# nv-dvl/nerfmatch

Hardware: AMD Instinct MI355X
Metric: rays*samples/sec (higher is better)
Workload: dtype fp16x3 (fp16 MFMA on hi/lo-split fp32 operands, three products per fp32 product, fp32 accumulate; fp32 everywhere else)

## Files before the change

### nerfmatch_amd/csrc/nerf_fwd_bf16.hip

```cpp
#include "nerf_split_chain.h"

namespace {
using namespace nmbf;

template <int PART>
__device__ __forceinline__ void tap_prefetch(Ctx& cx) {
  if constexpr (PART == 0) __builtin_amdgcn_s_barrier();
  const char* src = reinterpret_cast<const char*>(cx.tapw);
#pragma unroll
  for (int q = (PART == 0 ? 0 : 4); q < (PART == 0 ? 4 : 7); ++q) {
    const char* sp = src + q * 4096;
    const float* dp = q < 4 ? cx.tap_ring + q * 1024 : cx.tap_ipe + (q - 4) * 1024;
    const unsigned lds = (unsigned)__builtin_amdgcn_readfirstlane((int)(unsigned)(size_t)(const __attribute__((address_space(3))) float*)dp);
    unsigned m0_saved;
    asm volatile("s_mov_b32 %0, m0\n\ts_mov_b32 m0, %1\n\tglobal_load_lds_dwordx4 %2, off\n\tglobal_load_lds_dwordx4 %2, off offset:1024\n\t"
                 "global_load_lds_dwordx4 %2, off offset:2048\n\tglobal_load_lds_dwordx4 %2, off offset:3072\n\ts_mov_b32 m0, %0"
                 : "=&s"(m0_saved) : "s"(lds), "v"(sp) : "memory");
  }
}

__device__ __forceinline__ void dpp_pairs8(float (&o)[8], const float (&x)[8], const float (&y)[8], bool eight) {
  if (eight)
    asm("s_nop 1\n"
        "v_add_f32_dpp %0, %8, %8 row_mirror row_mask:0xf bank_mask:0x3\n\tv_add_f32_dpp %1, %9, %9 row_mirror row_mask:0xf bank_mask:0x3\n\t"
// ... 166 lines not shown
  const float o0 = rp[0], o1 = rp[1], o2 = rp[2], d0 = rp[3], d1 = rp[4], d2 = rp[5], radius = rp[11];
  const float dsq0 = d0 * d0, dsq1 = d1 * d1, dsq2 = d2 * d2;
  const float dmag = fmaxf(1e-10f, (dsq0 + dsq1) + dsq2);
  const float dnorm = sqrtf((dsq0 + dsq1) + dsq2);
  const float nul0 = 1.0f - dsq0 / dmag, nul1 = 1.0f - dsq1 / dmag, nul2 = 1.0f - dsq2 / dmag;

  float red_acc = 0.f;
  float carryT = 1.f;
  float best_w = -1.f;
  float feat_run = 0.f;

  const int nch = lo_pass ? 1 : nchunks;
  for (int chunk = 0; chunk < nch; ++chunk) {
    const int sidx = lo_pass ? Sa : chunk * TILE + (js % SP);
    const float t0 = a.t[(size_t)rc * (S + 1) + sidx];
    const float t1 = a.t[(size_t)rc * (S + 1) + sidx + 1];
    const float mu = (t0 + t1) / 2.0f, hw = (t1 - t0) / 2.0f;
    const float mu2 = mu * mu, hw2 = hw * hw, hw4 = hw2 * hw2;
    const float denom = fmaxf(1.1920928955078125e-07f, 3.0f * mu2 + hw2);
    const float t_mean = mu + (2.0f * mu * hw2) / denom;
    const float t_var = hw2 / 3.0f - (float)(4.0 / 15.0) * ((hw4 * (12.0f * mu2 - hw2)) / (denom * denom));
    const float r_var = (radius * radius) * ((mu2 / 4.0f + (float)(5.0 / 12.0) * hw2) - (float)(4.0 / 15.0) * hw4 / denom);
    float mean[3] = {d0 * t_mean + o0, d1 * t_mean + o1, d2 * t_mean + o2};
    float var[3] = {t_var * dsq0 + r_var * nul0, t_var * dsq1 + r_var * nul1, t_var * dsq2 + r_var * nul2};
    if (a.var_scale > 0.f) {
      var[0] *= a.var_scale; var[1] *= a.var_scale; var[2] *= a.var_scale;
    }
    if (hi == 0) {
      sm_t0[js] = t0; sm_t1[js] = t1;
      sm_mean[js] = mean[0]; sm_mean[TILE + js] = mean[1]; sm_mean[2 * TILE + js] = mean[2];
      sm_dn[js] = dnorm;
    }

#pragma unroll
    for (int g0 = 0; g0 < ring_ahead<P>(); ++g0) dma_slot<P>(blob_slots, g0, ring, wave, lane);

    {
      float* dst = sm_ipe + wave * (XS * 2 * 64 * 4) + lane * 4;
      const float ipe_scale = sm_small[OFF_INSCALE];
      const float phl = hi ? 1.57079637050628662109375f : 0.f;
#pragma unroll
      for (int m = 0; m < XS; ++m) {
        float v8[8];
#pragma unroll
        for (int i = 0; i < 8; ++i) {
          const int idx = 8 * m + i;
          const bool live = idx < 45;
          const int ax = (live ? idx : 0) % 3, sb = (live ? idx : 0) / 3;
          const float mu = mean[ax], vr = var[ax];
          const float sc = (float)(1 << sb);
          const float xe = mu * sc;
          float v = __builtin_amdgcn_exp2f((-0.5f * (vr * (sc * sc))) * 1.44269504088896340736f) * sin32(xe + phl);
          if constexpr (P == 2) v *= ipe_scale;
          v8[i] = live ? v : 0.f;
        }
        if constexpr (is_split<P>()) {
          bf16x8 h8, l8;
          split8_p<P>(v8, h8, l8);
          *reinterpret_cast<u32x4*>(dst + (m * 2 + 0) * 256) = __builtin_bit_cast(u32x4, h8);
          *reinterpret_cast<u32x4*>(dst + (m * 2 + 1) * 256) = __builtin_bit_cast(u32x4, l8);
        } else {
          *reinterpret_cast<u32x4*>(dst + m * 256) = __builtin_bit_cast(u32x4, pack8_f16(v8));
        }
      }
    }

    TRACE(2);
    Ctx cx;
    cx.blob_slots = blob_slots; cx.ring = ring; cx.sm_small = sm_small;
    cx.tapw = reinterpret_cast<f32x4*>(a.ws) + ((size_t)blockIdx.x * 4 + wave) * 32 * 64 + lane;
    cx.nslots = nslots; cx.wave = wave; cx.lane = lane; cx.hi = hi; cx.tap = need_tap ? tap : -1; cx.g = 0; cx.sig_part = 0.f;
    cx.vmax = 0.f; cx.rng = sm_rng + tid; cx.sc = 1.f;
    const bool early = need_rgb && !lo_pass && tap == 7 && a.feat && !a.sfeat;
    cx.tap_pref = need_tap && !lo_pass && !early; cx.rgb = need_rgb;
    cx.tap_ring = ring + wave * SLOT_FLOATS; cx.tap_ipe = sm_ipe + wave * (XS * 2 * 64 * 4);
    if constexpr (is_split<P>()) {
      NM_WAIT_VMCNT(8);
      __builtin_amdgcn_s_barrier();
    } else {
      ring_acquire<P>(blob_slots, 0, nslots, ring, wave, lane);
    }
    load_half<P>(cx.opA, ring, lane, 0);
    if constexpr (P == 1) load_half<1>(cx.opB, ring, lane, 1);
    const float* ipe_src = sm_ipe + wave * (XS * 2 * 64 * 4) + lane * 4;

    auto composite_weights = [&]() __attribute__((always_inline)) {
      const int tid2 = launder(threadIdx.x), lane2 = tid2 & 63, wave2 = tid2 >> 6;
      float alpha = 0.f, incl = 1.f;
      if (tid2 < TILE) {
        const float sg = fmaxf(sm_sigma[tid2], 0.f);
        const float delta = (sm_t1[tid2] - sm_t0[tid2]) * sm_dn[tid2];
        alpha = 1.0f - expf(-sg * delta);
        incl = (1.0f - alpha) + 1e-10f;
        const int seg = SP < 64 ? SP : 64;
#pragma unroll
        for (int dlt = 1; dlt < 64; dlt <<= 1) {
          const float up = __shfl_up(incl, dlt, 64);
          if (dlt < seg && (lane2 & (seg - 1)) >= dlt) incl *= up;
        }
        if (lane2 == 63) sm_misc[wave2] = incl;
      }
      NM_EPI_BARRIER();
      if (tid2 < TILE) {
        const int seg = SP < 64 ? SP : 64;
        float excl = __shfl_up(incl, 1, 64);
        if ((lane2 & (seg - 1)) == 0) excl = 1.f;
        if (SP == TILE && wave2 == 1) excl *= sm_misc[0];
        excl *= carryT;
        sm_w[tid2] = alpha * excl;
        const int r2 = tid2 / SP, ray2 = bid * nr + r2;
        if (left && chunk == nchunks - 1 && ray2 < R && tid2 % SP == SP - 1) {
// ... 102 lines not shown
      views_hidden<P>(av, cx);
      fold_range<P>(cx, 7);
      bf16x8 exh[VS], exl[VS];
#pragma unroll
      for (int e = 0; e < VS; ++e) {
        float v8[8];
        if (!lo_pass) {
          const f32x4 e0 = *reinterpret_cast<const f32x4*>(exr + 16 * e), e1 = *reinterpret_cast<const f32x4*>(exr + 16 * e + 4);
          v8[0] = e0[0]; v8[1] = e0[1]; v8[2] = e0[2]; v8[3] = e0[3]; v8[4] = e1[0]; v8[5] = e1[1]; v8[6] = e1[2]; v8[7] = e1[3];
        } else {
          const float* rq = a.rays + (size_t)launder(rc) * 12 + 8;
          const float vd0 = rq[0], vd1 = rq[1], vd2 = rq[2];
#pragma unroll
          for (int i = 0; i < 8; ++i) {
            const int f = 16 * e + 8 * hh + i;
            const int ax = f % 3;
            const float dax = ax == 0 ? vd0 : ax == 1 ? vd1 : vd2;
            float v = 0.f;
            if (f < 24) {
              const float xe = dax * (float)(1 << ((f % 12) / 3));
              v = nm_sinf(f < 12 ? xe : xe + 1.57079637050628662109375f);
            } else if (f < 27) {
              v = dax;
            } else if (f < 43) {
              v = a.app_row ? a.app_row[f - 27] : 0.f;
            }
            if constexpr (P == 2) v *= sm_small[OFF_INSCALE + (f < 27 ? 1 : 2)];
            v8[i] = v;
          }
        }
        if constexpr (is_split<P>()) split8_p<P>(v8, exh[e], exl[e]);
        else exh[e] = exl[e] = pack8_f16(v8);
      }
      views_extras<P>(av, cx, exh, exl);
      TRACE(11);
      NM_MLP_DONE_WAIT();
      if (cx.tap_pref) tap_prefetch<0>(cx);
      const float* bv = sm_small + OFF_BVIEWS + 4 * hh;
      const float* wr = sm_small + OFF_WRGB + 4 * hh;
      float pr = 0.f, pg = 0.f, pb = 0.f;
#pragma unroll
      for (int ob = 0; ob < 4; ++ob) {
#pragma unroll
        for (int q = 0; q < 4; ++q) {
          const f32x4 b4 = *reinterpret_cast<const f32x4*>(bv + ob * 32 + 8 * q);
          const f32x4 wr4 = *reinterpret_cast<const f32x4*>(wr + ob * 32 + 8 * q);
          const f32x4 wg4 = *reinterpret_cast<const f32x4*>(wr + 128 + ob * 32 + 8 * q);
          const f32x4 wb4 = *reinterpret_cast<const f32x4*>(wr + 256 + ob * 32 + 8 * q);
#pragma unroll
          for (int e = 0; e < 4; ++e) {
            const float hv = __builtin_fmaxf(acc_read(av[ob][4 * q + e]) + b4[e], 0.f);
            pr = NM_FMA(hv, wr4[e], pr);
            pg = NM_FMA(hv, wg4[e], pg);
            pb = NM_FMA(hv, wb4[e], pb);
          }
        }
      }
      pr = (pr + nm_shfl_xor32(pr)) + sm_small[OFF_MISC + 1];
      pg = (pg + nm_shfl_xor32(pg)) + sm_small[OFF_MISC + 2];
      pb = (pb + nm_shfl_xor32(pb)) + sm_small[OFF_MISC + 3];
      c_r = 1.0f / (1.0f + expf(-pr));
      c_g = 1.0f / (1.0f + expf(-pg));
      c_b = 1.0f / (1.0f + expf(-pb));
      if (cx.tap_pref) tap_prefetch<1>(cx);
    }
    const float sigma_raw = (cx.sig_part + nm_shfl_xor32(cx.sig_part)) + sm_small[OFF_MISC];
    TRACE(12);
// ... 240 lines not shown
```

### nerfmatch_amd/csrc/nerf_points_bf16.hip

```cpp
#include "nerf_split_chain.h"

namespace {
using namespace nmbf;

struct PointsArgs {
  const char* blob;
  const float* xi;
  const float* xd;
  const float* g4;
  float* out4;
  float* g_xi0;
  float* g_xi5;
  float* g_xd;
  u32x4* gates;
  int n, ntiles;
  const float* rays;
  const float* z;
  const float* app_row;
  int S, Sa;
  float* feats;
  const float* tap_w;
  const float* tap_g;
  int tap;
};

__device__ __forceinline__ void dump_tap_rows(int lo, const Ctx& cx, float* dst_row, int hh, bool valid) {
  const float* bl = cx.sm_small + OFF_BIAS + lo * 256 + 4 * hh;
  auto* tp = (__attribute__((address_space(1))) f32x4*)(dst_row + 4 * hh);
#pragma unroll
  for (int ob = 0; ob < 8; ++ob)
#pragma unroll
    for (int q = 0; q < 4; ++q) {
      const f32x4 b = *reinterpret_cast<const f32x4*>(bl + ob * 32 + 8 * q);
      f32x4 v;
#pragma unroll
      for (int e = 0; e < 4; ++e) v[e] = __builtin_fmaxf(cx.hv[ob * 16 + 4 * q + e] + b[e], 0.f);
      if (valid) tp[ob * 8 + q * 2] = v;
    }
}

template <int P, bool RAYS>
__device__ __forceinline__ void points_fwd_body(const PointsArgs& a) {
  __shared__ __attribute__((aligned(16))) float sm[LDS_SCR];
  float* const sm_small = sm + LDS_SMALL;
  float* const ring = sm + LDS_RING;
  float* const sm_ipe = sm + LDS_IPE;
  const int tid = threadIdx.x, lane = tid & 63, wave = tid >> 6, s = lane & 31, hi = lane >> 5;
  const char* const blob_slots = a.blob + (size_t)SMALL_PAD * 4;
  for (int i = tid; i < SMALL / 4; i += 256) reinterpret_cast<f32x4*>(sm_small)[i] = reinterpret_cast<const f32x4*>(a.blob)[i];
#pragma unroll 1
  for (int bid = blockIdx.x; bid < a.ntiles; bid += gridDim.x) {
    __syncthreads();
    const int sample = bid * TILE + wave * 32 + s;
    const size_t sc = (size_t)(sample < a.n ? sample : a.n - 1);
#pragma unroll
    for (int g0 = 0; g0 < ring_ahead<P>(); ++g0) dma_slot<P>(blob_slots, g0, ring, wave, lane);
    float vdir[3] = {0.f, 0.f, 0.f};
    {
      float* dst = sm_ipe + wave * (XS * 2 * 64 * 4) + lane * 4;
      if constexpr (RAYS) {
        const int r = (int)(sc / (size_t)a.Sa), si = (int)(sc % (size_t)a.Sa);
        const float* rp = a.rays + (size_t)r * 12;
        const float t0 = a.z[(size_t)r * (a.S + 1) + si], t1 = a.z[(size_t)r * (a.S + 1) + si + 1];
        const float d0 = rp[3], d1 = rp[4], d2 = rp[5], radius = rp[11];
        vdir[0] = rp[8]; vdir[1] = rp[9]; vdir[2] = rp[10];
        const float mu = (t0 + t1) / 2.0f, hw = (t1 - t0) / 2.0f;
        const float mu2 = mu * mu, hw2 = hw * hw, hw4 = hw2 * hw2;
        const float denom = fmaxf(1.1920928955078125e-07f, 3.0f * mu2 + hw2);
        const float t_mean = mu + (2.0f * mu * hw2) / denom;
        const float t_var = hw2 / 3.0f - (float)(4.0 / 15.0) * ((hw4 * (12.0f * mu2 - hw2)) / (denom * denom));
        const float r_var = (radius * radius) * ((mu2 / 4.0f + (float)(5.0 / 12.0) * hw2) - (float)(4.0 / 15.0) * hw4 / denom);
        const float dsq[3] = {d0 * d0, d1 * d1, d2 * d2};
        const float dmag = fmaxf(1e-10f, (dsq[0] + dsq[1]) + dsq[2]);
        float mean[3], var[3];
#pragma unroll
        for (int ax = 0; ax < 3; ++ax) {
          mean[ax] = rp[ax] + t_mean * vdir[ax];
          var[ax] = t_var * dsq[ax] + r_var * (1.0f - dsq[ax] / dmag);
        }
        const float phl = hi ? 1.57079637050628662109375f : 0.f;
#pragma unroll
        for (int m = 0; m < XS; ++m) {
          float v8[8];
#pragma unroll
          for (int i = 0; i < 8; ++i) {
            const int idx = 8 * m + i;
            const bool live = idx < 45;
            const int ax = (live ? idx : 0) % 3, sb = (live ? idx : 0) / 3;
            const float scl = (float)(1 << sb);
            const float xe = mean[ax] * scl;
            const float v = expf(-0.5f * (var[ax] * (scl * scl))) * nm_sinf(xe + phl);
            v8[i] = live ? v : 0.f;
          }
          bf16x8 h8, l8;
          split8_p<P>(v8, h8, l8);
          *reinterpret_cast<u32x4*>(dst + (m * 2 + 0) * 256) = __builtin_bit_cast(u32x4, h8);
          *reinterpret_cast<u32x4*>(dst + (m * 2 + 1) * 256) = __builtin_bit_cast(u32x4, l8);
        }
      } else {
        const float* row = a.xi + sc * 96 + 45 * hi;
#pragma unroll
        for (int m = 0; m < XS; ++m) {
          float v8[8];
#pragma unroll
          for (int i = 0; i < 8; ++i) v8[i] = (8 * m + i) < 45 ? row[8 * m + i] : 0.f;
          bf16x8 h8, l8;
          split8_p<P>(v8, h8, l8);
          *reinterpret_cast<u32x4*>(dst + (m * 2 + 0) * 256) = __builtin_bit_cast(u32x4, h8);
          *reinterpret_cast<u32x4*>(dst + (m * 2 + 1) * 256) = __builtin_bit_cast(u32x4, l8);
        }
      }
    }
    Ctx cx;
    cx.blob_slots = blob_slots; cx.ring = ring; cx.sm_small = sm_small; cx.tapw = nullptr;
    cx.nslots = NSLOT_FULL; cx.wave = wave; cx.lane = lane; cx.hi = hi; cx.tap = -1; cx.g = 0; cx.sig_part = 0.f;
    cx.vmax = 0.f; cx.rng = nullptr; cx.sc = 1.f; cx.tap_pref = false; cx.rgb = true; cx.tap_ring = nullptr; cx.tap_ipe = nullptr;
    cx.gptr = a.gates + (size_t)bid * 9 * 256 + tid;
    cx.gbits[0] = cx.gbits[1] = cx.gbits[2] = cx.gbits[3] = 0u;
    NM_WAIT_VMCNT(8);
    __builtin_amdgcn_s_barrier();
    load_half<P>(cx.opA, ring, lane, 0);
    const float* ipe_src = sm_ipe + wave * (XS * 2 * 64 * 4) + lane * 4;
    f32x16 acc[8];
    ipe_steps<P, true>(acc, cx, ipe_src);
    finish_layer<P>(acc, 0, cx);
    const bool tapped = a.feats != nullptr;
#pragma unroll 1
    for (int l = 1; l < 8; ++l) {
      if (tapped && l - 1 == a.tap) dump_tap_rows(l - 1, cx, a.feats + sc * 256, launder(lane) >> 5, sample < a.n);
      layer_pass<P>(acc, l, cx, ipe_src);
    }
    if (tapped && a.tap == 7) dump_tap_rows(7, cx, a.feats + sc * 256, launder(lane) >> 5, sample < a.n);
    f32x16 av[4];
    views_hidden<P>(av, cx);
    cx.gptr[7 * 256] = u32x4{cx.gbits[0], cx.gbits[1], cx.gbits[2], cx.gbits[3]};
    const int hh = launder(lane) >> 5;
    {
      const float* row = a.xd + sc * 48 + 8 * hh;
      bf16x8 exh[VS], exl[VS];
#pragma unroll
      for (int e = 0; e < VS; ++e) {
        float v8[8];
        if constexpr (RAYS) {
#pragma unroll
          for (int i = 0; i < 8; ++i) {
            const int f = 16 * e + 8 * hh + i;
            const int ax = f % 3;
            const float dax = ax == 0 ? vdir[0] : ax == 1 ? vdir[1] : vdir[2];
            float v = 0.f;
            if (f < 24) {
              const float xe = dax * (float)(1 << ((f % 12) / 3));
              v = nm_sinf(f < 12 ? xe : xe + 1.57079637050628662109375f);
            } else if (f < 27) {
              v = dax;
            } else if (f < 43) {
              v = a.app_row ? a.app_row[f - 27] : 0.f;
            }
            v8[i] = v;
          }
        } else {
          const f32x4 e0 = *reinterpret_cast<const f32x4*>(row + 16 * e), e1 = *reinterpret_cast<const f32x4*>(row + 16 * e + 4);
          v8[0] = e0[0]; v8[1] = e0[1]; v8[2] = e0[2]; v8[3] = e0[3]; v8[4] = e1[0]; v8[5] = e1[1]; v8[6] = e1[2]; v8[7] = e1[3];
        }
        split8_p<P>(v8, exh[e], exl[e]);
      }
      views_extras<P>(av, cx, exh, exl);
    }
    const float* bv = sm_small + OFF_BVIEWS + 4 * hh;
    const float* wr = sm_small + OFF_WRGB + 4 * hh;
    float pr = 0.f, pg = 0.f, pb = 0.f;
    unsigned gv0 = 0u, gv1 = 0u;
#pragma unroll
    for (int ob = 0; ob < 4; ++ob)
#pragma unroll
      for (int q = 0; q < 4; ++q) {
        const f32x4 b4 = *reinterpret_cast<const f32x4*>(bv + ob * 32 + 8 * q);
        const f32x4 wr4 = *reinterpret_cast<const f32x4*>(wr + ob * 32 + 8 * q);
        const f32x4 wg4 = *reinterpret_cast<const f32x4*>(wr + 128 + ob * 32 + 8 * q);
        const f32x4 wb4 = *reinterpret_cast<const f32x4*>(wr + 256 + ob * 32 + 8 * q);
#pragma unroll
        for (int e = 0; e < 4; ++e) {
          const float hv = __builtin_fmaxf(acc_read(av[ob][4 * q + e]) + b4[e], 0.f);
          const unsigned bit = min(__float_as_uint(hv), 1u) << (16 * (ob & 1) + 4 * q + e);
          if (ob < 2) gv0 |= bit; else gv1 |= bit;
          pr = NM_FMA(hv, wr4[e], pr);
          pg = NM_FMA(hv, wg4[e], pg);
          pb = NM_FMA(hv, wb4[e], pb);
        }
      }
    cx.gptr[8 * 256] = u32x4{gv0, gv1, 0u, 0u};
    pr = (pr + nm_shfl_xor32(pr)) + sm_small[OFF_MISC + 1];
    pg = (pg + nm_shfl_xor32(pg)) + sm_small[OFF_MISC + 2];
    pb = (pb + nm_shfl_xor32(pb)) + sm_small[OFF_MISC + 3];
    const float sigma_raw = (cx.sig_part + nm_shfl_xor32(cx.sig_part)) + sm_small[OFF_MISC];
    if (hh == 0 && sample < a.n) *reinterpret_cast<f32x4*>(a.out4 + (size_t)sample * 4) = f32x4{pr, pg, pb, sigma_raw};
  }
}

template <bool GATED>
// ... 74 lines not shown
    }
  }
}
__device__ __forceinline__ void take_acc8(const f32x16 (&acc)[8], Ctx& cx) {
#pragma unroll
  for (int ob = 0; ob < 8; ++ob)
#pragma unroll
    for (int r = 0; r < 16; ++r) cx.hv[ob * 16 + r] = acc_read(acc[ob][r]);
}
__device__ __forceinline__ void store_acc4(const f32x16 (&av)[4], float* dst_row, int ncol, int hh, bool valid) {
#pragma unroll
  for (int ob = 0; ob < 4; ++ob)
#pragma unroll
    for (int q = 0; q < 4; ++q) {
      const int c = 32 * ob + 8 * q + 4 * hh;
      const f32x4 v = {acc_read(av[ob][4 * q + 0]), acc_read(av[ob][4 * q + 1]), acc_read(av[ob][4 * q + 2]), acc_read(av[ob][4 * q + 3])};
      if (valid && c + 3 < ncol) *reinterpret_cast<f32x4*>(dst_row + c) = v;
    }
}

__device__ __forceinline__ void points_bwd_body(const PointsArgs& a) {
  __shared__ __attribute__((aligned(16))) float sm[LDS_IPE];
  float* const sm_small = sm + LDS_SMALL;
  float* const ring = sm + LDS_RING;
  const int tid = threadIdx.x, lane = tid & 63, wave = tid >> 6, s = lane & 31, hi = lane >> 5;
  const char* const blob_slots = a.blob + (size_t)SMALL_PAD * 4;
  for (int i = tid; i < SMALL / 4; i += 256) reinterpret_cast<f32x4*>(sm_small)[i] = reinterpret_cast<const f32x4*>(a.blob)[i];
#pragma unroll 1
  for (int bid = blockIdx.x; bid < a.ntiles; bid += gridDim.x) {
    __syncthreads();
    const int sample = bid * TILE + wave * 32 + s;
    const bool valid = sample < a.n;
    const size_t sc = (size_t)(valid ? sample : a.n - 1);
#pragma unroll
    for (int g0 = 0; g0 < ring_ahead<0>(); ++g0) dma_slot<0>(blob_slots, g0, ring, wave, lane);
    const u32x4* gt = a.gates + (size_t)bid * 9 * 256 + tid;
    const f32x4 g4 = *reinterpret_cast<const f32x4*>(a.g4 + sc * 4);
    Ctx cx;
    cx.blob_slots = blob_slots; cx.ring = ring; cx.sm_small = sm_small; cx.tapw = nullptr;
    cx.nslots = NSLOT_BWD; cx.wave = wave; cx.lane = lane; cx.hi = hi; cx.tap = -1; cx.g = launder_s(0); cx.sig_part = 0.f;
    cx.vmax = 0.f; cx.rng = nullptr; cx.sc = 1.f; cx.tap_pref = false; cx.rgb = true; cx.tap_ring = nullptr; cx.tap_ipe = nullptr; cx.gptr = nullptr;
    const int hh = launder(lane) >> 5;
    {
      const u32x4 gv = gt[8 * 256];
      const float* wr = sm_small + OFF_WRGB + 4 * hh;
#pragma unroll
      for (int ob = 0; ob < 4; ++ob)
#pragma unroll
        for (int q = 0; q < 4; ++q) {
          const f32x4 wr4 = *reinterpret_cast<const f32x4*>(wr + ob * 32 + 8 * q);
          const f32x4 wg4 = *reinterpret_cast<const f32x4*>(wr + 128 + ob * 32 + 8 * q);
          const f32x4 wb4 = *reinterpret_cast<const f32x4*>(wr + 256 + ob * 32 + 8 * q);
#pragma unroll
          for (int e = 0; e < 4; ++e) {
            const float g = NM_FMA(wb4[e], g4[2], NM_FMA(wg4[e], g4[1], wr4[e] * g4[0]));
            const int bit = 16 * (ob & 1) + 4 * q + e;
            cx.hv[ob * 16 + 4 * q + e] = __int_as_float(__float_as_int(g) & __builtin_amdgcn_sbfe((int)gv[ob >> 1], bit, 1));
          }
        }
    }
    NM_WAIT_VMCNT(8);
    __builtin_amdgcn_s_barrier();
    load_half<0>(cx.opA, ring, lane, 0);
    const u32x4 none = {0u, 0u, 0u, 0u};
    f32x16 acc[8];
    {
      f32x16 av[4];
      make_unit0_b<false>(cx, none);
      bwd_product<4, 8, false>(av, cx, none);
      store_acc4(av, a.g_xd + sc * 48, 48, hh, valid);
    }
    make_unit0_b<false>(cx, none);
    bwd_product<8, 8, false>(acc, cx, none);
    take_acc8(acc, cx);
    {
      const float* wa = sm_small + OFF_WALPHA + 4 * hh;
#pragma unroll
      for (int ob = 0; ob < 8; ++ob)
#pragma unroll
        for (int q = 0; q < 4; ++q) {
          const f32x4 w4v = *reinterpret_cast<const f32x4*>(wa + ob * 32 + 8 * q);
#pragma unroll
          for (int e = 0; e < 4; ++e) cx.hv[ob * 16 + 4 * q + e] = NM_FMA(w4v[e], g4[3], cx.hv[ob * 16 + 4 * q + e]);
        }
    }
#pragma unroll 1
    for (int l = 7; l >= 0; --l) {
      const u32x4 gw = gt[l * 256];
      if (l == a.tap && a.tap_g) {
        const float wn = valid ? a.tap_w[sc] : 0.f;
        const float* gr = a.tap_g + (sc / (size_t)a.Sa) * 256 + 4 * hh;
#pragma unroll
        for (int ob = 0; ob < 8; ++ob)
#pragma unroll
          for (int q = 0; q < 4; ++q) {
// ... 73 lines not shown
```

### nerfmatch_amd/csrc/nerf_split_chain.h

```cpp
#pragma once
#include "nerf_bf16_common.h"

namespace nmbf {

template <int P> constexpr bool is_bf16() { return P == 0 || P == 4; }
template <int P> constexpr bool has_gates() { return P == 4; }
typedef _Float16 f16x8 __attribute__((ext_vector_type(8)));
typedef _Float16 f16x2 __attribute__((ext_vector_type(2)));
template <int P>
__device__ __forceinline__ f32x16 mfma_p(const bf16x8& a, const bf16x8& b, const f32x16& c) {
  if constexpr (is_bf16<P>()) return MFMA_BF16(a, b, c);
  else return __builtin_amdgcn_mfma_f32_32x32x16_f16(__builtin_bit_cast(f16x8, a), __builtin_bit_cast(f16x8, b), c, 0, 0, 0);
}
template <int P> constexpr bool is_split() { return P != 1; }
template <int P> constexpr int slot_bytes() { return is_split<P>() ? SLOT_BYTES : SLOT_BYTES / 2; }
template <int P> constexpr int slot_floats() { return slot_bytes<P>() / 4; }
template <int P> constexpr int ring_slots() { return is_split<P>() ? NRING : 2 * NRING; }
template <int P> constexpr int ring_ahead() { return is_split<P>() ? 4 : 6; }
constexpr float F16_MAX = 65504.0f;
__device__ __forceinline__ void split8_f16(const float (&v)[8], bf16x8& hi, bf16x8& lo) {
  f16x8 h8, l8;
#pragma unroll
  for (int i = 0; i < 8; ++i) {
    const float c = __builtin_amdgcn_fmed3f(v[i], -F16_MAX, F16_MAX);
// ... 15 lines not shown
  const f16x2 h = {(_Float16)a, (_Float16)b};
  return __builtin_bit_cast(unsigned, h);
}
__device__ __forceinline__ bf16x8 pack8_f16(const float (&v)[8]) {
  const u32x4 r = {pack_f16(v[0], v[1]), pack_f16(v[2], v[3]), pack_f16(v[4], v[5]), pack_f16(v[6], v[7])};
  return __builtin_bit_cast(bf16x8, r);
}

template <int P>
__device__ __forceinline__ void dma_slot(const char* blob_slots, int g, float* ring, int wave, int lane) {
  const unsigned voff = (unsigned)(wave * (slot_bytes<P>() / 4) + lane * 16);
  const char* base = blob_slots + (size_t)g * slot_bytes<P>();
  const auto* src = (const __attribute__((address_space(1))) void*)(base + voff);
  auto* dst = (__attribute__((address_space(3))) void*)(ring_slot<P>(ring, g) + wave * (slot_floats<P>() / 4));
  __builtin_amdgcn_global_load_lds(src, dst, 16, 0, 0);
  __builtin_amdgcn_global_load_lds(src, dst, 16, 1024, 0);
  if constexpr (is_split<P>()) {
    __builtin_amdgcn_global_load_lds(src, dst, 16, 2048, 0);
    __builtin_amdgcn_global_load_lds(src, dst, 16, 3072, 0);
  }
}

template <int P>
__device__ __forceinline__ void ring_acquire(const char* blob_slots, int g, int nslots, float* ring, int wave, int lane) {
  if constexpr (is_split<P>()) {
    NM_WAIT_VMCNT(4);
  } else {
    NM_WAIT_VMCNT(10);
  }
  __builtin_amdgcn_s_barrier();
  if constexpr (is_split<P>()) dma_slot<P>(blob_slots, g + ring_ahead<P>(), ring, wave, lane);
}

template <int P>
__device__ __forceinline__ void ring_acquire_two(const char* blob_slots, int g, float* ring, int wave, int lane) {
  asm volatile("s_waitcnt vmcnt(0) lgkmcnt(0)" ::: "memory");
  __builtin_amdgcn_s_barrier();
  dma_slot<P>(blob_slots, g + 3, ring, wave, lane);
  dma_slot<P>(blob_slots, g + 4, ring, wave, lane);
}

__device__ __forceinline__ void ring_acquire_pair(const char* blob_slots, int g, float* ring, int wave, int lane) {
  NM_WAIT_VMCNT(6);
  __builtin_amdgcn_s_barrier();
  dma_slot<1>(blob_slots, g + 6, ring, wave, lane);
  dma_slot<1>(blob_slots, g + 7, ring, wave, lane);
}

struct OpHalf {
  bf16x8 h[4], l[4];
};

template <int P>
__device__ __forceinline__ void load_half(OpHalf& d, const float* slot, int lane, int p) {
  const u32x4* s4 = reinterpret_cast<const u32x4*>(slot) + lane;
#pragma unroll
  for (int o = 0; o < 4; ++o) {
    if constexpr (is_split<P>()) {
      d.h[o] = __builtin_bit_cast(bf16x8, s4[((4 * p + o) * 2 + 0) * 64]);
      d.l[o] = __builtin_bit_cast(bf16x8, s4[((4 * p + o) * 2 + 1) * 64]);
    } else {
      d.h[o] = __builtin_bit_cast(bf16x8, s4[(4 * p + o) * 64]);
    }
  }
}

struct Ctx {
  const char* blob_slots;
  float* ring;
  const float* sm_small;
  f32x4* tapw;
  bool tap_pref;
  bool rgb;
  float* tap_ring;
  float* tap_ipe;
  int nslots, wave, lane, hi;
  int tap;
  int g;
  OpHalf opA;
  OpHalf opB;
  Unit xn;
  float sig_part;
  float sc;
  float vmax;
  unsigned* rng;
  u32x4* gptr;
  unsigned gbits[4];
  float hv[128];
};

__device__ __forceinline__ unsigned gate_byte(const u32x4& h) {
  const unsigned w0 = h[0], w1 = h[1], w2 = h[2], w3 = h[3];
  unsigned m0, m1, m2, m3;
  const unsigned one = 0x00010001u;
  asm("v_pk_min_u16 %0, %1, %2" : "=v"(m0) : "v"(w0), "v"(one));
  asm("v_pk_min_u16 %0, %1, %2" : "=v"(m1) : "v"(w1), "v"(one));
  asm("v_pk_min_u16 %0, %1, %2" : "=v"(m2) : "v"(w2), "v"(one));
  asm("v_pk_min_u16 %0, %1, %2" : "=v"(m3) : "v"(w3), "v"(one));
  const unsigned t = m0 | (m1 << 1) | (m2 << 2) | (m3 << 3);
  return (t & 0xfu) | ((t >> 12) & 0xf0u);
}

template <int P>
struct UnitWork {
  Ctx& cx;
  Unit& out;
  int u, lo;
  float floor_v;
  f32x4 b0, b1;
  float sc;
  float v8[8];
  float f0, f1;
  unsigned hpk;
  __device__ __forceinline__ void prefetch() {
    const int ob = u >> 1, m = u & 1;
    const float* bl = cx.sm_small + OFF_BIAS + lo * 256 + ob * 32 + 16 * m + 4 * cx.hi;
    b0 = *reinterpret_cast<const f32x4*>(bl); b1 = *reinterpret_cast<const f32x4*>(bl + 8);
  }
  __device__ __forceinline__ void operator()(int j) {
    const int ob = u >> 1, m = u & 1;
    if (j < 4) {
      if constexpr (is_bf16<P>()) {
// ... 162 lines not shown
  if constexpr (ACQ) ring_acquire_pair(cx.blob_slots, g, cx.ring, cx.wave, cx.lane);
  NM_SB;
  acc[1] = mfma_p<1>(A.h[1], x, FIRST ? zero : acc[1]); NM_SB;
  cx.opA.h[0] = load_op1(nxt, cx.lane, 0); cx.opA.h[1] = load_op1(nxt, cx.lane, 1); work.prefetch(); NM_SB;
  acc[2] = mfma_p<1>(A.h[2], x, FIRST ? zero : acc[2]); NM_SB;
  cx.opA.h[2] = load_op1(nxt, cx.lane, 2); cx.opA.h[3] = load_op1(nxt, cx.lane, 3); NM_SB;
  acc[3] = mfma_p<1>(A.h[3], x, FIRST ? zero : acc[3]); NM_SB;
  cx.opB.h[0] = load_op1(nxt, cx.lane, 4); cx.opB.h[1] = load_op1(nxt, cx.lane, 5); NM_SB;
  acc[4] = mfma_p<1>(B.h[0], x, FIRST ? zero : acc[4]); NM_SB;
  cx.opB.h[2] = load_op1(nxt, cx.lane, 6); cx.opB.h[3] = load_op1(nxt, cx.lane, 7); NM_SB;
  acc[5] = mfma_p<1>(B.h[1], x, FIRST ? zero : acc[5]); NM_SB;
  work(0); work(1); NM_SB;
  acc[6] = mfma_p<1>(B.h[2], x, FIRST ? zero : acc[6]); NM_SB;
  work(2); work(3); work(4); NM_SB;
  acc[7] = mfma_p<1>(B.h[3], x, FIRST ? zero : acc[7]); NM_SB;
  work(5); work(6); work(7); NM_SB;
  cx.g = g + 1;
}

template <int P, bool FIRST, bool EVEN, class Work>
__device__ __forceinline__ void slot_step8(f32x16 (&acc)[8], Ctx& cx, const bf16x8& xh, const bf16x8& xl, Work work) {
  if constexpr (P == 1) {
    slot_step8_one<FIRST, EVEN>(acc, cx, xh, work);
    return;
  }
  const f32x16 zero = {0.f, 0.f, 0.f, 0.f, 0.f, 0.f, 0.f, 0.f, 0.f, 0.f, 0.f, 0.f, 0.f, 0.f, 0.f, 0.f};
  const int g = cx.g;
  OpHalf B;
  mfma_head<P, FIRST, 8>(acc, 0, cx.opA, xh);
  __builtin_amdgcn_sched_barrier(0);
  load_half<P>(B, cx.ring + (g & (NRING - 1)) * SLOT_FLOATS, cx.lane, 1);
  work.prefetch();
  __builtin_amdgcn_sched_barrier(0);
  mfma_tail<P, 8>(acc, 0, cx.opA, xh, xl);
  __builtin_amdgcn_sched_barrier(0);
  if constexpr (!EVEN) ring_acquire_two<P>(cx.blob_slots, g, cx.ring, cx.wave, cx.lane);
#pragma unroll
  for (int o = 0; o < 4; ++o) {
    acc[4 + o] = mfma_p<P>(B.h[o], xh, FIRST ? zero : acc[4 + o]);
    __builtin_amdgcn_sched_barrier(0);
    work(o);
    __builtin_amdgcn_sched_barrier(0);
  }
  load_half<P>(cx.opA, cx.ring + ((g + 1) & (NRING - 1)) * SLOT_FLOATS, cx.lane, 0);
  __builtin_amdgcn_sched_barrier(0);
#pragma unroll
  for (int o = 0; o < 4; ++o) {
    acc[4 + o] = mfma_p<P>(B.h[o], xl, acc[4 + o]);
    __builtin_amdgcn_sched_barrier(0);
    work(4 + o);
    __builtin_amdgcn_sched_barrier(0);
  }
#pragma unroll
  for (int o = 0; o < 4; ++o) {
    acc[4 + o] = mfma_p<P>(B.l[o], xh, acc[4 + o]);
    __builtin_amdgcn_sched_barrier(0);
    work(8 + o);
    __builtin_amdgcn_sched_barrier(0);
  }
  cx.g = g + 1;
}

template <bool FIRST, bool ACQ, class Work>
__device__ __forceinline__ void slot_step4_one(f32x16 (&acc)[4], Ctx& cx, const bf16x8& x, Work work) {
  const f32x16 zero = {0.f, 0.f, 0.f, 0.f, 0.f, 0.f, 0.f, 0.f, 0.f, 0.f, 0.f, 0.f, 0.f, 0.f, 0.f, 0.f};
  const int g = cx.g;
  const OpHalf C = cx.opA;
  const float* nxt = ring_slot<1>(cx.ring, g + 1);
  acc[0] = mfma_p<1>(C.h[0], x, FIRST ? zero : acc[0]); NM_SB;
  if constexpr (ACQ) ring_acquire_pair(cx.blob_slots, g, cx.ring, cx.wave, cx.lane);
  NM_SB;
  acc[1] = mfma_p<1>(C.h[1], x, FIRST ? zero : acc[1]); NM_SB;
#pragma unroll
  for (int o = 0; o < 4; ++o) cx.opA.h[o] = load_op1(nxt, cx.lane, o);
  work.prefetch(); NM_SB;
  acc[2] = mfma_p<1>(C.h[2], x, FIRST ? zero : acc[2]); NM_SB;
  work(0); work(1); work(2); work(3); NM_SB;
  acc[3] = mfma_p<1>(C.h[3], x, FIRST ? zero : acc[3]); NM_SB;
  work(4); work(5); work(6); work(7); NM_SB;
  cx.g = g + 1;
}

template <int P, bool FIRST, bool EVEN, class Work>
__device__ __forceinline__ void slot_step4(f32x16 (&acc)[4], Ctx& cx, const bf16x8& xh, const bf16x8& xl, Work work) {
  if constexpr (P == 1) {
    slot_step4_one<FIRST, EVEN>(acc, cx, xh, work);
    return;
  }
  const f32x16 zero = {0.f, 0.f, 0.f, 0.f, 0.f, 0.f, 0.f, 0.f, 0.f, 0.f, 0.f, 0.f, 0.f, 0.f, 0.f, 0.f};
  const int g = cx.g;
  const OpHalf C = cx.opA;
  work.prefetch();
  if constexpr (!EVEN) ring_acquire_two<P>(cx.blob_slots, g, cx.ring, cx.wave, cx.lane);
#pragma unroll
  for (int o = 0; o < 4; ++o) {
    acc[o] = mfma_p<P>(C.h[o], xh, FIRST ? zero : acc[o]);
    __builtin_amdgcn_sched_barrier(0);
    work(o);
    __builtin_amdgcn_sched_barrier(0);
  }
  load_half<P>(cx.opA, cx.ring + ((g + 1) & (NRING - 1)) * SLOT_FLOATS, cx.lane, 0);
  __builtin_amdgcn_sched_barrier(0);
#pragma unroll
  for (int o = 0; o < 4; ++o) {
    acc[o] = mfma_p<P>(C.h[o], xl, acc[o]);
    __builtin_amdgcn_sched_barrier(0);
    work(4 + o);
    __builtin_amdgcn_sched_barrier(0);
  }
#pragma unroll
  for (int o = 0; o < 4; ++o) {
    acc[o] = mfma_p<P>(C.l[o], xh, acc[o]);
    __builtin_amdgcn_sched_barrier(0);
    work(8 + o);
    __builtin_amdgcn_sched_barrier(0);
  }
  cx.g = g + 1;
}

template <int P, bool FIRST, bool EVEN, class W0, class W1>
__device__ __forceinline__ void slot_step4x2(f32x16 (&av)[4], Ctx& cx, const bf16x8& x0h, const bf16x8& x0l, Unit& u1, W0 w0, W1 w1) {
  const f32x16 zero = {0.f, 0.f, 0.f, 0.f, 0.f, 0.f, 0.f, 0.f, 0.f, 0.f, 0.f, 0.f, 0.f, 0.f, 0.f, 0.f};
  const int g = cx.g;
  const OpHalf A = cx.opA;
  OpHalf B;
  w0.prefetch();
#pragma unroll
  for (int o = 0; o < 4; ++o) {
    av[o] = mfma_p<P>(A.h[o], x0h, FIRST ? zero : av[o]);
    __builtin_amdgcn_sched_barrier(0);
    w0(o);
    __builtin_amdgcn_sched_barrier(0);
  }
  load_half<P>(B, cx.ring + (g & (NRING - 1)) * SLOT_FLOATS, cx.lane, 1);
  __builtin_amdgcn_sched_barrier(0);
#pragma unroll
  for (int o = 0; o < 4; ++o) {
    av[o] = mfma_p<P>(A.h[o], x0l, av[o]);
    __builtin_amdgcn_sched_barrier(0);
    w0(4 + o);
    __builtin_amdgcn_sched_barrier(0);
  }
#pragma unroll
  for (int o = 0; o < 4; ++o) {
    av[o] = mfma_p<P>(A.l[o], x0h, av[o]);
    __builtin_amdgcn_sched_barrier(0);
    w0(8 + o);
    __builtin_amdgcn_sched_barrier(0);
  }
  if constexpr (!EVEN) ring_acquire_two<P>(cx.blob_slots, g, cx.ring, cx.wave, cx.lane);
  const bf16x8 x1h = __builtin_bit_cast(bf16x8, u1.h), x1l = __builtin_bit_cast(bf16x8, u1.l);
  w1.prefetch();
#pragma unroll
  for (int o = 0; o < 4; ++o) {
    av[o] = mfma_p<P>(B.h[o], x1h, av[o]);
    __builtin_amdgcn_sched_barrier(0);
    w1(o);
    __builtin_amdgcn_sched_barrier(0);
  }
  load_half<P>(cx.opA, cx.ring + ((g + 1) & (NRING - 1)) * SLOT_FLOATS, cx.lane, 0);
  __builtin_amdgcn_sched_barrier(0);
#pragma unroll
  for (int o = 0; o < 4; ++o) {
    av[o] = mfma_p<P>(B.h[o], x1l, av[o]);
    __builtin_amdgcn_sched_barrier(0);
    w1(4 + o);
    __builtin_amdgcn_sched_barrier(0);
  }
#pragma unroll
  for (int o = 0; o < 4; ++o) {
    av[o] = mfma_p<P>(B.l[o], x1h, av[o]);
    __builtin_amdgcn_sched_barrier(0);
    w1(8 + o);
    __builtin_amdgcn_sched_barrier(0);
  }
  cx.g = g + 1;
}

template <int P>
__device__ __forceinline__ void views_hidden(f32x16 (&av)[4], Ctx& cx) {
  if constexpr (is_split<P>()) {
#pragma unroll
    for (int sl = 0; sl < HS / 2; ++sl) {
      const Unit x0 = cx.xn;
      Unit u1;
      const bf16x8 x0h = __builtin_bit_cast(bf16x8, x0.h), x0l = __builtin_bit_cast(bf16x8, x0.l);
      if (sl == 0) slot_step4x2<P, true, true>(av, cx, x0h, x0l, u1, unit_work<P>(1, 7, cx, u1), unit_work<P>(2, 7, cx, cx.xn));
      else if (sl + 1 == HS / 2) slot_step4x2<P, false, false>(av, cx, x0h, x0l, u1, unit_work<P>(2 * sl + 1, 7, cx, u1), NoWork{});
      else if (sl & 1) slot_step4x2<P, false, false>(av, cx, x0h, x0l, u1, unit_work<P>(2 * sl + 1, 7, cx, u1), unit_work<P>(2 * sl + 2, 7, cx, cx.xn));
      else slot_step4x2<P, false, true>(av, cx, x0h, x0l, u1, unit_work<P>(2 * sl + 1, 7, cx, u1), unit_work<P>(2 * sl + 2, 7, cx, cx.xn));
    }
  } else {
#pragma unroll
    for (int ks = 0; ks < HS; ks += 2) {
      {
        const Unit xc = cx.xn;
        if (ks == 0) slot_step4<P, true, true>(av, cx, __builtin_bit_cast(bf16x8, xc.h), __builtin_bit_cast(bf16x8, xc.l), unit_work<P>(ks + 1, 7, cx, cx.xn));
        else slot_step4<P, false, true>(av, cx, __builtin_bit_cast(bf16x8, xc.h), __builtin_bit_cast(bf16x8, xc.l), unit_work<P>(ks + 1, 7, cx, cx.xn));
      }
      {
        const Unit xc = cx.xn;
        if (ks + 2 < HS) slot_step4<P, false, false>(av, cx, __builtin_bit_cast(bf16x8, xc.h), __builtin_bit_cast(bf16x8, xc.l), unit_work<P>(ks + 2, 7, cx, cx.xn));
        else slot_step4<P, false, false>(av, cx, __builtin_bit_cast(bf16x8, xc.h), __builtin_bit_cast(bf16x8, xc.l), NoWork{});
      }
    }
  }
}
template <int P>
__device__ __forceinline__ void views_extras(f32x16 (&av)[4], Ctx& cx, const bf16x8 (&eh)[VS], const bf16x8 (&el)[VS]) {
  if constexpr (is_split<P>()) {
    Unit u1;
    u1.h = __builtin_bit_cast(u32x4, eh[1]); u1.l = __builtin_bit_cast(u32x4, el[1]);
    slot_step4x2<P, false, true>(av, cx, eh[0], el[0], u1, NoWork{}, NoWork{});
    slot_step4<P, false, false>(av, cx, eh[2], el[2], NoWork{});
  } else {
#pragma unroll
    for (int e = 0; e < VS; ++e) {
      if (e & 1) slot_step4<P, false, false>(av, cx, eh[e], el[e], NoWork{});
      else slot_step4<P, false, true>(av, cx, eh[e], el[e], NoWork{});
    }
  }
}

template <int P, bool FIRST>
__device__ __forceinline__ void ipe_steps(f32x16 (&acc)[8], Ctx& cx, const float* ipe_src) {
  auto operand = [&](int m, bf16x8& ph, bf16x8& pl) {
    ph = __builtin_bit_cast(bf16x8, *reinterpret_cast<const u32x4*>(ipe_src + (is_split<P>() ? (m * 2 + 0) : m) * 256));
    pl = ph;
    if constexpr (is_split<P>()) pl = __builtin_bit_cast(bf16x8, *reinterpret_cast<const u32x4*>(ipe_src + (m * 2 + 1) * 256));
  };
#pragma unroll
  for (int m = 0; m < XS; m += 2) {
    bf16x8 ph, pl;
    operand(m, ph, pl);
    if (m == 0) slot_step8<P, FIRST, true>(acc, cx, ph, pl, NoWork{});
    else slot_step8<P, false, true>(acc, cx, ph, pl, NoWork{});
    operand(m + 1, ph, pl);
    if (m + 2 == XS) slot_step8<P, false, false>(acc, cx, ph, pl, AccTake<P>{acc, cx});
    else slot_step8<P, false, false>(acc, cx, ph, pl, NoWork{});
  }
}

struct Tap7Workspace {
  static constexpr bool on = false;
  __device__ __forceinline__ void fn(Ctx&) const {}
};
template <class F>
struct Tap7InRegisters {
  bool on;
  F fn;
};

template <int P, class Tap7 = Tap7Workspace>
// ... 33 lines not shown
```

Baseline: 365.4 million.

## Interleave weight-ring DMA pieces with MFMAs and skip empty appearance slot

The ring prefetch is reworked. Only two slots are opened up front, and on even steps the next slots are requested in 1 KB pieces placed between individual MFMAs, using precomputed voffset/LDS bases kept in Ctx. Odd steps now only wait and barrier, where before they issued two full slot DMAs in a burst. The views stage also skips the third extras MFMA slot when there is no appearance row, since those inputs are zero. This risks desync in ring slot accounting, because skipping a slot step changes the g count, and the opening wait is now a full vmcnt(0).

Measured after the change: 375.8 million (median of 6 runs). +2.9%, better.

```diff
diff --git a/nerfmatch_amd/csrc/nerf_fwd_bf16.hip b/nerfmatch_amd/csrc/nerf_fwd_bf16.hip
--- a/nerfmatch_amd/csrc/nerf_fwd_bf16.hip
+++ b/nerfmatch_amd/csrc/nerf_fwd_bf16.hip
@@ -222,8 +222,7 @@
       sm_dn[js] = dnorm;
     }
 
-#pragma unroll
-    for (int g0 = 0; g0 < ring_ahead<P>(); ++g0) dma_slot<P>(blob_slots, g0, ring, wave, lane);
+    ring_open<P>(blob_slots, ring, wave, lane);
 
     {
       float* dst = sm_ipe + wave * (XS * 2 * 64 * 4) + lane * 4;
@@ -265,8 +264,7 @@
     cx.tap_pref = need_tap && !lo_pass && !early; cx.rgb = need_rgb;
     cx.tap_ring = ring + wave * SLOT_FLOATS; cx.tap_ipe = sm_ipe + wave * (XS * 2 * 64 * 4);
     if constexpr (is_split<P>()) {
-      NM_WAIT_VMCNT(8);
-      __builtin_amdgcn_s_barrier();
+      ring_open_wait<P>(cx);
     } else {
       ring_acquire<P>(blob_slots, 0, nslots, ring, wave, lane);
     }
@@ -435,7 +433,7 @@
         if constexpr (is_split<P>()) split8_p<P>(v8, exh[e], exl[e]);
         else exh[e] = exl[e] = pack8_f16(v8);
       }
-      views_extras<P>(av, cx, exh, exl);
+      views_extras<P>(av, cx, exh, exl, a.app_row == nullptr);
       TRACE(11);
       NM_MLP_DONE_WAIT();
       if (cx.tap_pref) tap_prefetch<0>(cx);
diff --git a/nerfmatch_amd/csrc/nerf_points_bf16.hip b/nerfmatch_amd/csrc/nerf_points_bf16.hip
--- a/nerfmatch_amd/csrc/nerf_points_bf16.hip
+++ b/nerfmatch_amd/csrc/nerf_points_bf16.hip
@@ -53,8 +53,7 @@
     __syncthreads();
     const int sample = bid * TILE + wave * 32 + s;
     const size_t sc = (size_t)(sample < a.n ? sample : a.n - 1);
-#pragma unroll
-    for (int g0 = 0; g0 < ring_ahead<P>(); ++g0) dma_slot<P>(blob_slots, g0, ring, wave, lane);
+    ring_open<P>(blob_slots, ring, wave, lane);
     float vdir[3] = {0.f, 0.f, 0.f};
     {
       float* dst = sm_ipe + wave * (XS * 2 * 64 * 4) + lane * 4;
@@ -117,8 +116,7 @@
     cx.vmax = 0.f; cx.rng = nullptr; cx.sc = 1.f; cx.tap_pref = false; cx.rgb = true; cx.tap_ring = nullptr; cx.tap_ipe = nullptr;
     cx.gptr = a.gates + (size_t)bid * 9 * 256 + tid;
     cx.gbits[0] = cx.gbits[1] = cx.gbits[2] = cx.gbits[3] = 0u;
-    NM_WAIT_VMCNT(8);
-    __builtin_amdgcn_s_barrier();
+    ring_open_wait<P>(cx);
     load_half<P>(cx.opA, ring, lane, 0);
     const float* ipe_src = sm_ipe + wave * (XS * 2 * 64 * 4) + lane * 4;
     f32x16 acc[8];
@@ -164,7 +162,7 @@
         }
         split8_p<P>(v8, exh[e], exl[e]);
       }
-      views_extras<P>(av, cx, exh, exl);
+      views_extras<P>(av, cx, exh, exl, RAYS && a.app_row == nullptr);
     }
     const float* bv = sm_small + OFF_BVIEWS + 4 * hh;
     const float* wr = sm_small + OFF_WRGB + 4 * hh;
@@ -305,8 +303,7 @@
     const int sample = bid * TILE + wave * 32 + s;
     const bool valid = sample < a.n;
     const size_t sc = (size_t)(valid ? sample : a.n - 1);
-#pragma unroll
-    for (int g0 = 0; g0 < ring_ahead<0>(); ++g0) dma_slot<0>(blob_slots, g0, ring, wave, lane);
+    ring_open<0>(blob_slots, ring, wave, lane);
     const u32x4* gt = a.gates + (size_t)bid * 9 * 256 + tid;
     const f32x4 g4 = *reinterpret_cast<const f32x4*>(a.g4 + sc * 4);
     Ctx cx;
@@ -332,8 +329,7 @@
           }
         }
     }
-    NM_WAIT_VMCNT(8);
-    __builtin_amdgcn_s_barrier();
+    ring_open_wait<0>(cx);
     load_half<0>(cx.opA, ring, lane, 0);
     const u32x4 none = {0u, 0u, 0u, 0u};
     f32x16 acc[8];
diff --git a/nerfmatch_amd/csrc/nerf_split_chain.h b/nerfmatch_amd/csrc/nerf_split_chain.h
--- a/nerfmatch_amd/csrc/nerf_split_chain.h
+++ b/nerfmatch_amd/csrc/nerf_split_chain.h
@@ -71,12 +71,9 @@
   if constexpr (is_split<P>()) dma_slot<P>(blob_slots, g + ring_ahead<P>(), ring, wave, lane);
 }
 
-template <int P>
-__device__ __forceinline__ void ring_acquire_two(const char* blob_slots, int g, float* ring, int wave, int lane) {
+__device__ __forceinline__ void ring_acquire_two() {
   asm volatile("s_waitcnt vmcnt(0) lgkmcnt(0)" ::: "memory");
   __builtin_amdgcn_s_barrier();
-  dma_slot<P>(blob_slots, g + 3, ring, wave, lane);
-  dma_slot<P>(blob_slots, g + 4, ring, wave, lane);
 }
 
 __device__ __forceinline__ void ring_acquire_pair(const char* blob_slots, int g, float* ring, int wave, int lane) {
@@ -116,6 +113,8 @@
   int nslots, wave, lane, hi;
   int tap;
   int g;
+  unsigned dma_voff;
+  unsigned dma_lds;
   OpHalf opA;
   OpHalf opB;
   Unit xn;
@@ -127,6 +126,37 @@
   unsigned gbits[4];
   float hv[128];
 };
+
+template <int P>
+__device__ __forceinline__ void ring_request(const Ctx& cx, int g, int j) {
+  const int slot = g + 2 + (j >> 2);
+  const char* base = cx.blob_slots + (size_t)slot * slot_bytes<P>();
+  const unsigned lds = cx.dma_lds + (unsigned)(slot & (ring_slots<P>() - 1)) * slot_bytes<P>();
+  unsigned m0_saved;
+#define NM_DMA_PIECE(OFS)                                                                                                        \
+  asm volatile("s_mov_b32 %0, m0\n\ts_mov_b32 m0, %1\n\tglobal_load_lds_dwordx4 %2, %3 offset:" #OFS "\n\ts_mov_b32 m0, %0" \
+               : "=&s"(m0_saved) : "s"(lds), "v"(cx.dma_voff), "s"(base) : "memory")
+  switch (j & 3) {
+    case 0: NM_DMA_PIECE(0); break;
+    case 1: NM_DMA_PIECE(1024); break;
+    case 2: NM_DMA_PIECE(2048); break;
+    default: NM_DMA_PIECE(3072); break;
+  }
+#undef NM_DMA_PIECE
+}
+template <int P>
+__device__ __forceinline__ void ring_open(const char* blob_slots, float* ring, int wave, int lane) {
+#pragma unroll
+  for (int g0 = 0; g0 < (is_split<P>() ? 2 : ring_ahead<P>()); ++g0) dma_slot<P>(blob_slots, g0, ring, wave, lane);
+}
+template <int P>
+__device__ __forceinline__ void ring_open_wait(Ctx& cx) {
+  cx.dma_voff = (unsigned)(cx.wave * (slot_bytes<P>() / 4) + cx.lane * 16);
+  const float* q = cx.ring + cx.wave * (slot_floats<P>() / 4);
+  cx.dma_lds = (unsigned)__builtin_amdgcn_readfirstlane((int)(unsigned)(size_t)(const __attribute__((address_space(3))) float*)q);
+  NM_WAIT_VMCNT(0);
+  __builtin_amdgcn_s_barrier();
+}
 
 __device__ __forceinline__ unsigned gate_byte(const u32x4& h) {
   const unsigned w0 = h[0], w1 = h[1], w2 = h[2], w3 = h[3];
@@ -355,9 +385,19 @@
   load_half<P>(B, cx.ring + (g & (NRING - 1)) * SLOT_FLOATS, cx.lane, 1);
   work.prefetch();
   __builtin_amdgcn_sched_barrier(0);
-  mfma_tail<P, 8>(acc, 0, cx.opA, xh, xl);
-  __builtin_amdgcn_sched_barrier(0);
-  if constexpr (!EVEN) ring_acquire_two<P>(cx.blob_slots, g, cx.ring, cx.wave, cx.lane);
+  if constexpr (EVEN) {
+#pragma unroll
+    for (int o = 0; o < 8; ++o) {
+      acc[o & 3] = mfma_p<P>(o < 4 ? cx.opA.h[o & 3] : cx.opA.l[o & 3], o < 4 ? xl : xh, acc[o & 3]);
+      ring_request<P>(cx, g, o);
+      __builtin_amdgcn_sched_barrier(0);
+    }
+  } else {
+    mfma_tail<P, 8>(acc, 0, cx.opA, xh, xl);
+    __builtin_amdgcn_sched_barrier(0);
+    ring_acquire_two();
+    __builtin_amdgcn_sched_barrier(0);
+  }
 #pragma unroll
   for (int o = 0; o < 4; ++o) {
     acc[4 + o] = mfma_p<P>(B.h[o], xh, FIRST ? zero : acc[4 + o]);
@@ -414,7 +454,7 @@
   const int g = cx.g;
   const OpHalf C = cx.opA;
   work.prefetch();
-  if constexpr (!EVEN) ring_acquire_two<P>(cx.blob_slots, g, cx.ring, cx.wave, cx.lane);
+  if constexpr (!EVEN) ring_acquire_two();
 #pragma unroll
   for (int o = 0; o < 4; ++o) {
     acc[o] = mfma_p<P>(C.h[o], xh, FIRST ? zero : acc[o]);
@@ -428,6 +468,7 @@
   for (int o = 0; o < 4; ++o) {
     acc[o] = mfma_p<P>(C.h[o], xl, acc[o]);
     __builtin_amdgcn_sched_barrier(0);
+    if constexpr (EVEN) ring_request<P>(cx, g, o);
     work(4 + o);
     __builtin_amdgcn_sched_barrier(0);
   }
@@ -435,6 +476,7 @@
   for (int o = 0; o < 4; ++o) {
     acc[o] = mfma_p<P>(C.l[o], xh, acc[o]);
     __builtin_amdgcn_sched_barrier(0);
+    if constexpr (EVEN) ring_request<P>(cx, g, 4 + o);
     work(8 + o);
     __builtin_amdgcn_sched_barrier(0);
   }
@@ -461,6 +503,7 @@
   for (int o = 0; o < 4; ++o) {
     av[o] = mfma_p<P>(A.h[o], x0l, av[o]);
     __builtin_amdgcn_sched_barrier(0);
+    if constexpr (EVEN) ring_request<P>(cx, g, o);
     w0(4 + o);
     __builtin_amdgcn_sched_barrier(0);
   }
@@ -468,10 +511,14 @@
   for (int o = 0; o < 4; ++o) {
     av[o] = mfma_p<P>(A.l[o], x0h, av[o]);
     __builtin_amdgcn_sched_barrier(0);
+    if constexpr (EVEN) ring_request<P>(cx, g, 4 + o);
     w0(8 + o);
     __builtin_amdgcn_sched_barrier(0);
   }
-  if constexpr (!EVEN) ring_acquire_two<P>(cx.blob_slots, g, cx.ring, cx.wave, cx.lane);
+  if constexpr (!EVEN) {
+    ring_acquire_two();
+    __builtin_amdgcn_sched_barrier(0);
+  }
   const bf16x8 x1h = __builtin_bit_cast(bf16x8, u1.h), x1l = __builtin_bit_cast(bf16x8, u1.l);
   w1.prefetch();
 #pragma unroll
@@ -530,18 +577,16 @@
   }
 }
 template <int P>
-__device__ __forceinline__ void views_extras(f32x16 (&av)[4], Ctx& cx, const bf16x8 (&eh)[VS], const bf16x8 (&el)[VS]) {
+__device__ __forceinline__ void views_extras(f32x16 (&av)[4], Ctx& cx, const bf16x8 (&eh)[VS], const bf16x8 (&el)[VS], bool no_app) {
   if constexpr (is_split<P>()) {
     Unit u1;
     u1.h = __builtin_bit_cast(u32x4, eh[1]); u1.l = __builtin_bit_cast(u32x4, el[1]);
     slot_step4x2<P, false, true>(av, cx, eh[0], el[0], u1, NoWork{}, NoWork{});
-    slot_step4<P, false, false>(av, cx, eh[2], el[2], NoWork{});
+    if (!no_app) slot_step4<P, false, false>(av, cx, eh[2], el[2], NoWork{});
   } else {
-#pragma unroll
-    for (int e = 0; e < VS; ++e) {
-      if (e & 1) slot_step4<P, false, false>(av, cx, eh[e], el[e], NoWork{});
-      else slot_step4<P, false, true>(av, cx, eh[e], el[e], NoWork{});
-    }
+    slot_step4<P, false, true>(av, cx, eh[0], el[0], NoWork{});
+    slot_step4<P, false, false>(av, cx, eh[1], el[1], NoWork{});
+    if (!no_app) slot_step4<P, false, true>(av, cx, eh[2], el[2], NoWork{});
   }
 }
 
```
